# gunesevitan/otto-multi-objective-recommender-system

Measured on AMD Instinct MI355X. Metric: aid-pairs/sec covisitation build, higher is better.
Workload: dtype u64

## Files before the change

otto-multi-objective-recommender-system_amd/csrc/otto_covis.hip:

```cpp
#include "common.h"
#include "topk.h"
#include "scan.h"
#include "../../include/otto_covis.h"

#include <stdarg.h>
#include <string.h>
#include <type_traits>
#include <vector>

namespace otto {

static thread_local std::string g_err;
void set_error(const char* fmt, ...) {
    char buf[1024];
    va_list ap;
    va_start(ap, fmt);
    vsnprintf(buf, sizeof buf, fmt, ap);
    va_end(ap);
    g_err = buf;
}

struct WinPairs {
    const int64_t* off;
    int W;
// ... 1473 lines not shown
__global__ __launch_bounds__(ORD_BLOCK) void k_ord_scatter(const uint64_t* keys, const uint64_t* chunks, uint32_t n, OrdBin dg,
                                                           uint32_t n_blocks, const uint64_t* cell_start, uint64_t* out) {
    __shared__ uint32_t s_bin[ORD_BLOCK];
    const uint32_t i = blockIdx.x * ORD_BLOCK + threadIdx.x;
    const uint32_t bin = i < n ? dg(keys[i]) : 0xffffffffu;
    s_bin[threadIdx.x] = bin;
    __syncthreads();
    if (i >= n) return;
    uint32_t rank = 0;
    for (uint32_t j = 0; j < threadIdx.x; ++j) rank += s_bin[j] == bin ? 1u : 0u;
    const uint64_t pos = cell_start[(size_t)bin * n_blocks + blockIdx.x] + rank;
    if (pos < n) out[pos] = chunks[i];
}

constexpr int N_TOTALS = 18;
constexpr int ITEM_BLOCK_AIDS = 2048;
constexpr int N_ITEM_SCANS = 10;
__global__ __launch_bounds__(256) void k_aid_totals(const uint64_t* cnt64, const uint8_t* boost, const uint32_t* flag, uint32_t n_aids,
                                                    uint32_t l_cap, int allow_packed, unsigned long long* totals,
                                                    unsigned long long* block_part) {
    __shared__ unsigned long long s_t[4][N_TOTALS];
    unsigned long long t[N_TOTALS];
#pragma unroll
    for (int q = 0; q < N_TOTALS; ++q) t[q] = 0;
    const uint32_t x_end = min(n_aids, (blockIdx.x + 1) * (uint32_t)ITEM_BLOCK_AIDS);
    for (uint32_t x = blockIdx.x * ITEM_BLOCK_AIDS + threadIdx.x; x < x_end; x += 256) {
        const uint64_t c64 = cnt64[x], n = c64 & CNT_REC_MASK, r = c64 >> CNT_REC_BITS;
        if (n == 0) continue;
        const int b = n <= (uint64_t)S_CAP ? 0 : (n <= (uint64_t)M_CAP ? 1 : 2);
        t[0] += n; t[1] += r; t[2 + b] += n; t[5 + b] += r;
        ItemCount f{cnt64, boost, flag, b, 0, l_cap, allow_packed, -1};
        const uint64_t items = f((int64_t)x);
        t[8 + b] += items;
        if (b == 2) {
            const int mode = heavy_mode(c64, allow_packed, l_cap);
            t[11 + mode] += items;
            t[14 + mode] += 1;
            ChunkCount cf{cnt64, boost, flag, 0, l_cap, allow_packed};
            t[17] += cf((int64_t)x);
        }
    }
#pragma unroll
    for (int q = 0; q < N_TOTALS; ++q) {
        unsigned long long v = t[q];
        for (int o = 32; o > 0; o >>= 1) v += __shfl_xor(v, o, 64);
        if (lane_id() == 0) s_t[threadIdx.x >> 6][q] = v;
    }
    __syncthreads();
    if (threadIdx.x < N_TOTALS) {
        const unsigned long long v = s_t[0][threadIdx.x] + s_t[1][threadIdx.x] + s_t[2][threadIdx.x] + s_t[3][threadIdx.x];
        if (v) atomicAdd(&totals[threadIdx.x], v);
        if (block_part && threadIdx.x >= N_TOTALS - N_ITEM_SCANS)
            block_part[(size_t)blockIdx.x * N_ITEM_SCANS + threadIdx.x - (N_TOTALS - N_ITEM_SCANS)] = v;
    }
}

struct ItemFillArgs {
    const uint64_t* cnt64;
    const uint8_t* boost;
    uint32_t n_aids;
    uint32_t l_cap;
    int allow_packed;
    const unsigned long long* block_part;
    uint64_t* items[3];
    uint32_t* order[3];
    uint64_t n_pilots[3];
    uint64_t* chunks;
    uint64_t* litem_start;
};
__global__ __launch_bounds__(64 * N_ITEM_SCANS) void k_item_part_scan(unsigned long long* block_part, uint32_t nblk) {
    const int q = threadIdx.x >> 6;
    const unsigned lane = lane_id();
    unsigned long long run = 0;
    for (uint32_t b0 = 0; b0 < nblk; b0 += 64) {
        const uint32_t b = b0 + lane;
        const unsigned long long v = b < nblk ? block_part[(size_t)b * N_ITEM_SCANS + q] : 0ull;
        const unsigned long long inc = wave_incl_scan(v);
        if (b < nblk) block_part[(size_t)b * N_ITEM_SCANS + q] = run + inc - v;
        run += (unsigned long long)__shfl((unsigned long long)inc, 63, 64);
    }
}

__global__ __launch_bounds__(256) void k_items_fill(ItemFillArgs a) {
    __shared__ unsigned long long s_base[N_ITEM_SCANS];
    __shared__ uint64_t s_sc[256 / 64 + 1];
    if (threadIdx.x < N_ITEM_SCANS) s_base[threadIdx.x] = a.block_part[(size_t)blockIdx.x * N_ITEM_SCANS + threadIdx.x];
    __syncthreads();
    uint64_t run[N_ITEM_SCANS];
#pragma unroll
    for (int q = 0; q < N_ITEM_SCANS; ++q) run[q] = s_base[q];
    for (int it = 0; it < ITEM_BLOCK_AIDS / 256; ++it) {
        const uint32_t x = blockIdx.x * ITEM_BLOCK_AIDS + it * 256 + threadIdx.x;
        int b = -1, mode = -1;
        uint64_t items = 0, nch = 0;
        if (x < a.n_aids) {
            const uint64_t c64 = a.cnt64[x], n = c64 & CNT_REC_MASK;
            if (n) {
                b = n <= (uint64_t)S_CAP ? 0 : (n <= (uint64_t)M_CAP ? 1 : 2);
                items = 1;
                if (b == 2) {
                    mode = heavy_mode(c64, a.allow_packed, a.l_cap);
                    const int lg = l_log2r(c64, a.boost[x], a.l_cap, a.allow_packed);
                    items = 1ull << lg;
                    if (lg) nch = ((c64 >> CNT_REC_BITS) + PART_CHUNK_RUNS - 1) / PART_CHUNK_RUNS;
                }
            }
        }
        const uint64_t small = (uint64_t)(b == 0) | (uint64_t)(b == 1) << 12 | (uint64_t)(mode == 0) << 24 | (uint64_t)(mode == 1) << 36 |
                               (uint64_t)(mode == 2) << 48;
        uint64_t tot_small, tot_l, tot_m[3], tot_c;
        const uint64_t ex_small = block_excl_scan<uint64_t, 256>(small, s_sc, &tot_small);
        const uint64_t ex_l = block_excl_scan<uint64_t, 256>(b == 2 ? items : 0ull, s_sc, &tot_l);
        uint64_t ex_m[3];
#pragma unroll
        for (int m = 0; m < 3; ++m) ex_m[m] = block_excl_scan<uint64_t, 256>(mode == m ? items : 0ull, s_sc, &tot_m[m]);
        const uint64_t ex_c = block_excl_scan<uint64_t, 256>(nch, s_sc, &tot_c);
        if (b == 0) a.items[0][run[0] + (ex_small & 0xFFF)] = (uint64_t)x;
        if (b == 1) a.items[1][run[1] + ((ex_small >> 12) & 0xFFF)] = (uint64_t)x;
        const uint64_t s = run[2] + ex_l;
        if (x < a.n_aids) a.litem_start[x] = s;
        if (x == a.n_aids - 1) a.litem_start[a.n_aids] = s + (b == 2 ? items : 0ull);
        if (b == 2) {
            uint64_t lg = 0;
            while ((1ull << lg) < items) ++lg;
            for (uint64_t p = 0; p < items; ++p) a.items[2][s + p] = (uint64_t)x | (p << 26) | (lg << 50);
            const uint64_t r = run[6 + mode] + ((ex_small >> (24 + 12 * mode)) & 0xFFF);
            const uint64_t sm = run[3 + mode] + ex_m[mode];
            uint32_t* ord = a.order[mode];
            ord[r] = (uint32_t)s;
            for (uint64_t p = 1; p < items; ++p) ord[a.n_pilots[mode] + sm + p - r - 1] = (uint32_t)(s + p);
            const uint64_t cs = run[9] + ex_c;
            for (uint64_t q = 0; q < nch; ++q) a.chunks[cs + q] = (uint64_t)x | (q << 26);
        }
        run[0] += tot_small & 0xFFF;
        run[1] += (tot_small >> 12) & 0xFFF;
        run[2] += tot_l;
#pragma unroll
        for (int m = 0; m < 3; ++m) {
            run[6 + m] += (tot_small >> (24 + 12 * m)) & 0xFFF;
            run[3 + m] += tot_m[m];
        }
        run[9] += tot_c;
    }
}

constexpr uint64_t TAB_EMPTY = ~0ull;

struct ItemDesc {
    uint32_t it;
    uint64_t item;
    uint64_t rb, re;
    uint64_t ps, pe;
};

#ifdef OTTO_PHASE_PROF
#define OTTO_PH(i) do { if (threadIdx.x == 0) { const unsigned long long _t = clock64(); ph[i] += _t - ph_t; ph_t = _t; } } while (0)
#else
#define OTTO_PH(i) do {} while (0)
#endif
template <int LOG2T, int THREADS, int GROUP, bool PACKED, int MINW, int GU, int INS_CH, bool DBG>
__global__ __launch_bounds__(THREADS, MINW) void k_reduce(ReduceArgs a) {
    constexpr int T = 1 << LOG2T;
    constexpr int NW = THREADS / 64;
    constexpr bool TP = GROUP == OTTO_COVIS_GROUP_TIME && PACKED;
    using K = typename std::conditional<GROUP == OTTO_COVIS_GROUP_TIME && !PACKED, KeyW, KeyN>::type;
    constexpr bool WIDE = GROUP == OTTO_COVIS_GROUP_TIME && !PACKED;
    auto kw = [](K key) -> uint64_t { if constexpr (TP) return key.c >> REC_AID_BITS; else return kweight(key); };
    constexpr bool DYNAMIC = true;
    constexpr int EXCAP = 64;
    constexpr int PKD = GROUP == OTTO_COVIS_GROUP_TIME ? 1 : PK;
    constexpr bool BOUND = GROUP == OTTO_COVIS_GROUP_TYPE && PKD > 1 && NW == 1;
    constexpr int CCAP = 256;
    constexpr bool HOT = NW > 1 && GROUP == OTTO_COVIS_GROUP_TYPE;
    __shared__ uint64_t s_tab[PACKED ? T : 1];
    __shared__ uint32_t s_key[PACKED ? 1 : T];
    __shared__ uint32_t s_v[3][PACKED ? 1 : T];
    constexpr int OCAP = NW == 1 ? 1 : (LOG2T == 12 ? 1920 : (LOG2T == 14 ? 10240 : (THREADS == 512 ? 4608 : 6144)));
    constexpr int RCAP = OCAP / NW;
    __shared__ uint16_t s_occ[OCAP];
    __shared__ uint32_t s_wcnt[NW];
    __shared__ uint32_t s_hcnt[NW];
    constexpr bool INWAVE = PACKED;
    __shared__ uint16_t s_lbi[(NW > 1 && !INWAVE) ? PKD : 1][(NW > 1 && !INWAVE) ? THREADS : 1];
    __shared__ uint64_t s_exw[(NW > 1 || BOUND) ? PKD : 1][(NW > 1 || BOUND) ? EXCAP : 1];
    __shared__ uint16_t s_cand[BOUND ? CCAP : 1];
    __shared__ uint32_t s_exy[1][(NW > 1 && WIDE) ? EXCAP : 1];
    __shared__ uint64_t s_thrw[PK];
    __shared__ uint32_t s_thry[PK];
    __shared__ uint32_t s_nex[PK];
    __shared__ uint32_t s_more;
    __shared__ uint32_t s_ovf;
    constexpr int LISTCAP = BOUND ? S_CAP : 256;
    __shared__ uint16_t s_list[NW == 1 ? LISTCAP : 1];
    __shared__ uint8_t s_seg[NW * 256 + 32];
    __shared__ ItemDesc s_cur;
    __shared__ ItemDesc s_nxt;

    const int wid = threadIdx.x >> 6;
    const unsigned lane = lane_id();
    constexpr bool HANDOVER = THREADS == M_THREADS;
    const int swid = HANDOVER ? __builtin_amdgcn_readfirstlane(wid) : wid;
    const bool pipe = threadIdx.x == (HANDOVER ? (NW - 1) * 64 : 0);
#ifdef OTTO_PHASE_PROF
    unsigned long long ph[24] = {0, 0, 0, 0, 0, 0, 0, 0, 0, 0, 0, 0, 0, 0, 0, 0, 0, 0, 0, 0, 0, 0, 0, 0}, ph_t = clock64();
#endif

    auto fetch_item = [&](uint32_t idx, ItemDesc& d) {
        d.it = 0xFFFFFFFFu;
        d.item = 0ull;
        if (idx < a.n_work) {
            d.it = a.order ? a.order[idx] : idx;
            d.item = a.items[d.it];
        }
    };
    auto fetch_ranges = [&](ItemDesc& d) {
        d.rb = d.re = d.ps = d.pe = 0;
        if (d.it != 0xFFFFFFFFu) {
            const uint32_t xx = (uint32_t)(d.item & REC_AID_MASK);
            d.rb = a.run_start[xx];
            d.re = a.run_start[xx + 1];
            if ((d.item >> 50) != 0 && a.pstart) {
                d.ps = a.pstart[d.it];
                const uint64_t cap = a.pstart[d.it + 1] - d.ps, got = a.pcursor[d.it];
                d.pe = d.ps + (got < cap ? got : cap);
            }
        }
    };
    ItemDesc cur, nx;
    uint32_t idx_next = 0, idx_far = 0;
    constexpr uint32_t DQ = THREADS == S_THREADS ? 16 : 4;
    uint32_t pool = 0, pool_end = 0, pool_next = 0;
    auto take = [&]() {
        const uint32_t r = pool++;
        if (pool == pool_end) {
            pool = pool_next;
            pool_end = pool + DQ;
            pool_next = atomicAdd(a.work_counter, DQ);
        }
        return r;
    };
    if (DYNAMIC) {
        if (pipe) {
            pool = atomicAdd(a.work_counter, 2 * DQ);
            pool_end = pool + DQ;
            pool_next = pool + DQ;
            const uint32_t i0 = take();
            idx_next = take();
            idx_far = take();
            fetch_item(i0, cur);
            fetch_ranges(cur);
            s_cur = cur;
        }
    } else {
        fetch_item(blockIdx.x, cur);
        fetch_ranges(cur);
    }
    uint32_t sidx = blockIdx.x;
    auto clear_slot = [&](int i) {
        if (PACKED) {
            s_tab[PACKED ? i : 0] = TAB_EMPTY;
        } else {
            s_key[PACKED ? 0 : i] = KEY_EMPTY;
            s_v[0][PACKED ? 0 : i] = 0; s_v[1][PACKED ? 0 : i] = 0; s_v[2][PACKED ? 0 : i] = 0;
        }
    };
    auto clear_table = [&]() {
        for (int i = threadIdx.x; i < T; i += THREADS) clear_slot(i);
    };
    if (NW > 1) {
        clear_table();
        if (threadIdx.x == 0) s_ovf = 0;
    }
    constexpr int BU = GROUP == OTTO_COVIS_GROUP_TIME ? 4 : ((PACKED && THREADS == L_THREADS) ? 12 : 6);
    constexpr bool PREF = THREADS == L_THREADS && GROUP != OTTO_COVIS_GROUP_TIME;
    constexpr bool WARM = (THREADS == L_THREADS || THREADS == 512) && GROUP != OTTO_COVIS_GROUP_TIME;
    uint32_t pre[PREF ? BU : 1];
    bool pre_valid = false;
    auto prefetch_next = [&]() {
        if (!PREF) return;
        const uint64_t nitem = s_nxt.item;
        pre_valid = s_nxt.it != 0xFFFFFFFFu && (nitem >> 50) != 0 && a.pstart != nullptr;
        if (!pre_valid) return;
        const uint64_t ps = s_nxt.ps, pe = s_nxt.pe;
#pragma unroll
        for (int u = 0; u < (PREF ? BU : 1); ++u) {
            const uint64_t i = ps + threadIdx.x + (uint64_t)u * THREADS;
            pre[u] = i < pe ? a.prec[i] : KEY_EMPTY;
        }
    };

    for (;;) {
        if (DYNAMIC) {
            __syncthreads();
            cur = s_cur;
        }
        if (cur.it == 0xFFFFFFFFu) break;
        OTTO_PH(0);
        const uint32_t it = cur.it;
        if (DYNAMIC) {
            if (pipe) fetch_item(idx_next, nx);
#ifdef OTTO_PHASE_PROF
            if (threadIdx.x == 0) { const unsigned long long _t = clock64(); ph[13] += _t - ph_t; }
#endif
        } else {
            fetch_item(sidx + gridDim.x, nx);
        }
        const uint64_t item = cur.item;
        const uint32_t x = (uint32_t)(item & REC_AID_MASK);
        const uint32_t part = (uint32_t)((item >> 26) & 0xFFFFFFu);
        constexpr bool CAN_PART = THREADS != M_THREADS;
        const int lgR = CAN_PART ? (int)(item >> 50) : 0;
        const uint32_t pmask = (1u << lgR) - 1u;
        const int pshift = 32 - LOG2T - lgR;

        K guess[PKD];
        const bool use_guess = NW > 1 && lgR > 0 && a.tau_w != nullptr;
#pragma unroll
        for (int j = 0; j < PKD; ++j) {
            kclear(guess[j]);
            if (use_guess && j < (BOUND ? 1 : a.nk)) {
                const size_t o = (size_t)j * a.n_aids + x;
                kload(guess[j], a.tau_w[o], WIDE ? a.tau_y[o] : 0u);
            }
        }
        if (NW == 1 && !(DBG && (a.debug_skip & 4))) clear_table();
        if (NW == 1) {
            s_ovf = 0;
            wave_lds_sync();
        }
        OTTO_PH(1);

        auto probe_step = [&](uint32_t y) -> uint32_t { return (((y * 0x85EBCA6Bu) ^ (y >> 7)) * 0xC2B2AE35u >> (32 - LOG2T)) | 1u; };
        uint32_t wc = 0;
        auto note_new = [&](uint64_t m, uint32_t slot) {
            if (NW == 1) return;
            if (m == 0) return;
            const uint32_t pos = wc + __builtin_amdgcn_mbcnt_hi((uint32_t)(m >> 32), __builtin_amdgcn_mbcnt_lo((uint32_t)m, 0u));
            if (__builtin_amdgcn_inverse_ballot_w64(m) && pos < (uint32_t)RCAP) s_occ[NW > 1 ? wid * RCAP + pos : 0] = (uint16_t)slot;
            wc += (uint32_t)__popcll(m);
        };
        constexpr int ICMP_EQ = 32, ICMP_NE = 33;
        auto probe_on = [&](uint32_t y, uint32_t slot, unsigned long long add, unsigned long long fresh) -> uint32_t {
            const uint32_t step = probe_step(y);
            for (int probe = 1; probe < T; ++probe) {
                slot = (slot + step) & (T - 1);
                const unsigned long long old = atomicCAS((unsigned long long*)&s_tab[PACKED ? slot : 0], (unsigned long long)TAB_EMPTY, fresh | add);
                if (old == TAB_EMPTY) return slot;
                if ((uint32_t)(old >> 36) == y) {
                    atomicAdd((unsigned long long*)&s_tab[PACKED ? slot : 0], add);
                    return 0xFFFFFFFFu;
                }
            }
            s_ovf = 1;
            return 0xFFFFFFFFu;
        };
        auto wide_add = [&](uint32_t rc, uint32_t found, uint32_t e) {
            if (GROUP == OTTO_COVIS_GROUP_TIME) {
                atomicAdd(&s_v[0][PACKED ? 0 : found], 1u);
                const uint32_t old = atomicAdd(&s_v[1][PACKED ? 0 : found], e);
                if (old + e < old) atomicAdd(&s_v[2][PACKED ? 0 : found], 1u);
            } else if (GROUP == OTTO_COVIS_GROUP_TYPE) {
                const uint32_t tyj = (rc >> REC_AID_BITS) & 3u;
                if (tyj < 3u) atomicAdd(&s_v[tyj][PACKED ? 0 : found], 1u);
            } else {
                const uint32_t fb = (rc >> 28) >> a.chan_shift;
                if (fb & 1u) atomicAdd(&s_v[0][PACKED ? 0 : found], 1u);
                if (fb & 2u) atomicAdd(&s_v[1][PACKED ? 0 : found], 1u);
                if (fb & 4u) atomicAdd(&s_v[2][PACKED ? 0 : found], 1u);
            }
        };
        auto packed_add = [&](uint32_t rc, uint32_t e) -> unsigned long long {
            uint32_t add0, add1, add2;
            if (GROUP == OTTO_COVIS_GROUP_TIME) {
                return 65536ull + (unsigned long long)e;
            } else if (GROUP == OTTO_COVIS_GROUP_TYPE) {
                const uint32_t tyj = (rc >> REC_AID_BITS) & 3u;
                return (unsigned long long)((1u << ((tyj * 12u) & 31u)) & 0x01001001u);
            } else {
                const uint32_t fb = (rc >> 28) >> a.chan_shift;
                add0 = fb & 1u; add1 = (fb >> 1) & 1u; add2 = (fb >> 2) & 1u;
            }
            return (unsigned long long)add0 | ((unsigned long long)add1 << 12) | ((unsigned long long)add2 << 24);
        };
        auto insert_batch = [&](auto ntag, const uint32_t* rc, const uint64_t* okin, const uint32_t* e) {
            constexpr int N = decltype(ntag)::value;
            constexpr int CH = INS_CH;
            if (DBG && (a.debug_skip & 8)) {
#pragma unroll
                for (int u = 0; u < N; ++u)
                    if (__builtin_amdgcn_inverse_ballot_w64(okin[u]) && rc[u] == 0xDEADBEEFu) s_ovf = 1;
                return;
            }
#pragma unroll
            for (int c0 = 0; c0 < N; c0 += CH) {
                bool ok[CH];
                uint64_t okm[CH];
                uint64_t any = 0;
#pragma unroll
                for (int q = 0; q < CH; ++q) {
                    const int u = c0 + q;
                    uint64_t m = u < N ? okin[u < N ? u : 0] : 0ull;
                    if (GROUP == OTTO_COVIS_GROUP_FILTER) m &= __builtin_amdgcn_uicmp(((rc[u < N ? u : 0] >> 28) >> a.chan_shift) & 7u, 0u, ICMP_NE);
                    okm[q] = m;
                    ok[q] = __builtin_amdgcn_inverse_ballot_w64(m);
                    any |= m;
                }
                if (any == 0) continue;
                if (PACKED) {
                    uint32_t oldhi[CH];
                    unsigned long long addq[CH];
#pragma unroll
                    for (int q = 0; q < CH; ++q) {
                        const uint32_t r = rc[c0 + q < N ? c0 + q : 0];
                        const uint32_t slot = rec_hash(r) >> (32 - LOG2T);
                        oldhi[q] = 0xFFFFFFFFu;
                        addq[q] = packed_add(r, e[c0 + q < N ? c0 + q : 0]);
                        if (ok[q]) {
                            const unsigned long long o = atomicCAS((unsigned long long*)&s_tab[PACKED ? slot : 0], (unsigned long long)TAB_EMPTY,
                                                                   ((unsigned long long)(r & REC_AID_MASK) << 36) | addq[q]);
                            oldhi[q] = (uint32_t)(o >> 32);
                        }
                        note_new(okm[q] & __builtin_amdgcn_uicmp(oldhi[q], 0xFFFFFFFFu, ICMP_EQ), slot);
                    }
#pragma unroll
                    for (int q = 0; q < CH; ++q) {
                        const uint32_t r = rc[c0 + q < N ? c0 + q : 0];
                        const uint32_t y = r & REC_AID_MASK, slot = rec_hash(r) >> (32 - LOG2T);
                        uint32_t late = 0xFFFFFFFFu;
                        if (oldhi[q] != 0xFFFFFFFFu) {
                            if ((oldhi[q] >> 4) == y) atomicAdd((unsigned long long*)&s_tab[PACKED ? slot : 0], addq[q]);
                            else late = probe_on(y, slot, addq[q], (unsigned long long)y << 36);
                        }
                        note_new(__builtin_amdgcn_uicmp(late, 0xFFFFFFFFu, ICMP_NE), late);
                    }
                    continue;
                }
                uint32_t old[CH];
#pragma unroll
                for (int q = 0; q < CH; ++q) {
                    const uint32_t r = rc[c0 + q < N ? c0 + q : 0];
                    old[q] = KEY_EMPTY;
                    if (ok[q]) old[q] = atomicCAS(&s_key[PACKED ? 0 : rec_hash(r) >> (32 - LOG2T)], KEY_EMPTY, r & REC_AID_MASK);
                    note_new(okm[q] & __builtin_amdgcn_uicmp(old[q], KEY_EMPTY, ICMP_EQ), rec_hash(r) >> (32 - LOG2T));
                }
#pragma unroll
                for (int q = 0; q < CH; ++q) {
                    const uint32_t r = rc[c0 + q < N ? c0 + q : 0];
                    const uint32_t y = r & REC_AID_MASK;
                    uint32_t sl = rec_hash(r) >> (32 - LOG2T);
                    uint32_t late = 0xFFFFFFFFu;
                    if (ok[q]) {
                        bool found = old[q] == KEY_EMPTY || old[q] == y;
                        const uint32_t step = probe_step(y);
                        for (int probe = 1; !found && probe < T; ++probe) {
                            sl = (sl + step) & (T - 1);
                            const uint32_t o2 = atomicCAS(&s_key[PACKED ? 0 : sl], KEY_EMPTY, y);
                            if (o2 == KEY_EMPTY) late = sl;
                            found = o2 == KEY_EMPTY || o2 == y;
                        }
                        if (!found) s_ovf = 1;
                        else wide_add(r, sl, e[c0 + q < N ? c0 + q : 0]);
                    }
                    note_new(__builtin_amdgcn_uicmp(late, 0xFFFFFFFFu, ICMP_NE), late);
                }
            }
        };

        auto slot_keys = [&](int i, K (&out)[PKD]) {
            uint32_t y, v0, v1, v2;
            if (PACKED) {
                const uint64_t v = s_tab[i];
                y = v == TAB_EMPTY ? KEY_EMPTY : (uint32_t)(v >> 36);
                v0 = (uint32_t)v & 0xFFFu; v1 = (uint32_t)(v >> 12) & 0xFFFu; v2 = (uint32_t)(v >> 24) & 0xFFFu;
            } else {
                y = s_key[i];
                v0 = s_v[0][i]; v1 = s_v[1][i]; v2 = s_v[2][i];
// ... 239 lines not shown
                        uint16_t sl = 0;
                        if (li < nvalid) {
                            K kl, kh;
                            sl = s_list[NW == 1 ? li : 0];
                            slot_lohi((int)sl, kl, kh);
                            c = !kbetter(thr, kh);
                        }
                        const uint64_t m = __ballot(c);
                        const uint32_t pos = ncand + __builtin_amdgcn_mbcnt_hi((uint32_t)(m >> 32), __builtin_amdgcn_mbcnt_lo((uint32_t)m, 0u));
                        if (c && pos < (uint32_t)CCAP) s_cand[pos] = sl;
                        ncand += (uint32_t)__popcll(m);
                    }
                    overflow = ncand > (uint32_t)CCAP;
                }
                wave_lds_sync();
                for (int j = 0; j < a.nk; ++j) {
                    if (overflow) wave_exact_topk(j);
                    else finish_kind(j, ncand);
                }
                wave_lds_sync();
            }
        }
        OTTO_PH(4);
        } else if constexpr (NW == 1) {
        bool fast_done = false;
        OTTO_PH(7);
        if (fast_done || (DBG && (a.debug_skip & 2))) {
        } else if (ovf) {
            if (threadIdx.x == 0) {
                a.flag[x] = 1;
                a.boost[x] = (uint8_t)(lgR - l_log2r(a.cnt64[x], 0, a.l_cap, a.allow_packed) + 1);
                atomicAdd(a.ovf_count, 1u);
            }
        } else {
            constexpr int MPL = T / THREADS;
            static_assert(MPL <= 32, "consumed-slot bitmask is 32 bits");
            bool compact_done = false;
            if (NW == 1) {
                uint32_t nvalid = 0;
#pragma unroll
                for (int q = 0; q < MPL; ++q) {
                    const int i = q * THREADS + threadIdx.x;
                    const bool v = PACKED ? (s_tab[PACKED ? i : 0] != TAB_EMPTY) : (s_key[PACKED ? 0 : i] != KEY_EMPTY);
                    const uint64_t m = __ballot(v);
                    const uint32_t pos = nvalid + __builtin_amdgcn_mbcnt_hi((uint32_t)(m >> 32), __builtin_amdgcn_mbcnt_lo((uint32_t)m, 0u));
                    if (v && pos < (uint32_t)LISTCAP) s_list[pos] = (uint16_t)i;
                    nvalid += (uint32_t)__popcll(m);
                }
                auto select_from_registers = [&](auto mtag) {
                    constexpr int MC = decltype(mtag)::value;
                    __syncthreads();
                    K c[PKD][MC];
#pragma unroll
                    for (int q = 0; q < MC; ++q) {
                        K kk[PKD];
#pragma unroll
                        for (int j = 0; j < PKD; ++j) kclear(kk[j]);
                        const uint32_t li = (uint32_t)q * 64u + lane;
                        if (li < nvalid) slot_keys((int)s_list[li], kk);
#pragma unroll
                        for (int j = 0; j < PKD; ++j) c[j][q] = kk[j];
                    }
                    K bests[PKD];
                    wave_topk_select_multi<MC, PKD, K>(c, a.nk, a.k, bests);
#pragma unroll
                    for (int j = 0; j < PKD; ++j)
                        if (j < a.nk) emit(j, bests[j]);
                    compact_done = true;
                    __syncthreads();
                };
                if (nvalid > 64u && nvalid <= 128u) select_from_registers(std::integral_constant<int, 2>{});
                else if (nvalid > 128u && nvalid <= 256u) select_from_registers(std::integral_constant<int, 4>{});
                if (nvalid <= 64u) {
                    __syncthreads();
                    K bests[PKD];
#pragma unroll
                    for (int j = 0; j < PKD; ++j) kclear(bests[j]);
                    if (lane < nvalid) slot_keys((int)s_list[lane], bests);
                    wave_bitonic_sort_multi<PKD, K>(bests);
#pragma unroll
                    for (int j = 0; j < PKD; ++j)
                        if (j < a.nk) emit(j, bests[j]);
                    compact_done = true;
                    __syncthreads();
                }
            }
            if (!compact_done) {
            K lb[PKD];
            uint32_t done[PKD];
            uint32_t nonempty = 0;
            {
                int bi[PKD];
#pragma unroll
                for (int j = 0; j < PKD; ++j) { kclear(lb[j]); bi[j] = 0; }
#pragma unroll 2
                for (int q = 0; q < MPL; ++q) {
                    K kk[PKD];
                    slot_keys(q * THREADS + threadIdx.x, kk);
                    bool any = false;
#pragma unroll
                    for (int j = 0; j < PKD; ++j) {
                        any = any || kvalid(kk[j]);
                        if (kbetter(kk[j], lb[j])) { lb[j] = kk[j]; bi[j] = q; }
                    }
                    if (any) nonempty |= 1u << q;
                }
#pragma unroll
                for (int j = 0; j < PKD; ++j) done[j] = 1u << bi[j];
            }
            if (NW == 1) {
                K bests[PKD];
#pragma unroll
                for (int j = 0; j < PKD; ++j) bests[j] = lb[j];
                wave_bitonic_sort_multi<PKD, K>(bests);
                for (;;) {
                    K thr[PKD], cb[PKD];
                    int ci[PKD];
#pragma unroll
                    for (int j = 0; j < PKD; ++j) {
                        thr[j] = kshfl(bests[j], a.k - 1);
                        kclear(cb[j]);
                        ci[j] = -1;
                    }
#pragma unroll 1
                    for (int q = 0; q < MPL; ++q) {
                        K kk[PKD];
                        slot_keys(q * THREADS + threadIdx.x, kk);
#pragma unroll
                        for (int j = 0; j < PKD; ++j)
                            if (!((done[j] >> q) & 1u) && kvalid(kk[j]) && kbetter(kk[j], thr[j]) &&
                                (ci[j] < 0 || kbetter(kk[j], cb[j]))) { cb[j] = kk[j]; ci[j] = q; }
                    }
                    bool any = false;
#pragma unroll
                    for (int j = 0; j < PKD; ++j) {
                        if (j >= a.nk) continue;
                        const bool qual = ci[j] >= 0;
                        if (__ballot(qual) == 0) continue;
                        any = true;
                        if (qual) done[j] |= 1u << ci[j];
                        wave_topk_push(bests[j], cb[j], a.k);
                    }
                    if (!any) break;
                }
#pragma unroll
                for (int j = 0; j < PKD; ++j)
                    if (j < a.nk) emit(j, bests[j]);
            }
            }
        }
        } else {
        const uint32_t nocc = s_wcnt[NW > 1 ? wid : 0];
        bool dense = true;
#pragma unroll
        for (int w = 0; w < NW; ++w) dense = dense && s_wcnt[NW > 1 ? w : 0] <= (uint32_t)RCAP;
        uint32_t nwalk = nocc;
        bool hot = false;
        if (HOT && dense && a.hot_ok) {
            constexpr int NITMAX = (RCAP + 63) / 64;
            uint32_t ent[NITMAX];
            uint32_t hv = 0, vv = 0;
            const int nq = (int)((nocc + 63u) / 64u);
#pragma unroll
            for (int q = 0; q < NITMAX; ++q) {
                const uint32_t idx = (uint32_t)q * 64u + lane;
                ent[q] = 0;
                if (q < nq && idx < nocc) {
                    const uint32_t sl = s_occ[NW > 1 ? wid * RCAP + idx : 0];
                    ent[q] = sl;
                    vv |= 1u << q;
                    bool light;
                    if (PACKED) light = (s_tab[PACKED ? sl : 0] & 0xFFFFFFFFFull) == 1ull;
                    else light = s_v[0][PACKED ? 0 : sl] == 1u && (s_v[1][PACKED ? 0 : sl] | s_v[2][PACKED ? 0 : sl]) == 0u;
                    if (!light) hv |= 1u << q;
                }
            }
            uint32_t H = 0;
#pragma unroll
            for (int q = 0; q < NITMAX; ++q)
                if (q < nq) H += (uint32_t)__popcll(__ballot((hv >> q) & 1u));
            uint32_t hpos = 0, lpos = H;
#pragma unroll
            for (int q = 0; q < NITMAX; ++q) {
                if (q < nq) {
                    const bool v = (vv >> q) & 1u, h = (hv >> q) & 1u;
                    const uint64_t mh = __ballot(h), ml = __ballot(v && !h);
                    if (v) {
                        const uint64_t m = h ? mh : ml;
                        const uint32_t pos = (h ? hpos : lpos) + __builtin_amdgcn_mbcnt_hi((uint32_t)(m >> 32), __builtin_amdgcn_mbcnt_lo((uint32_t)m, 0u));
                        s_occ[NW > 1 ? wid * RCAP + pos : 0] = (uint16_t)ent[q];
                    }
                    hpos += (uint32_t)__popcll(mh);
                    lpos += (uint32_t)__popcll(ml);
                }
            }
            if (lane == 0) s_hcnt[NW > 1 ? wid : 0] = H;
            wave_lds_sync();
            nwalk = H;
            hot = true;
        }
        if (ovf) {
            if (threadIdx.x == 0) {
                a.flag[x] = 1;
                a.boost[x] = (uint8_t)(lgR - l_log2r(a.cnt64[x], 0, a.l_cap, a.allow_packed) + 1);
                atomicAdd(a.ovf_count, 1u);
            }
        } else if (!(DBG && (a.debug_skip & 2))) {
            constexpr int MPL = T / THREADS;
            int nit = dense ? (int)((nwalk + 63u) / 64u) : MPL;
            auto slot_at = [&](int q) -> int {
                if (!dense) return q * THREADS + (int)threadIdx.x;
                const uint32_t idx = (uint32_t)q * 64u + lane;
                return idx < nwalk ? (int)s_occ[NW > 1 ? wid * RCAP + idx : 0] : -1;
            };
            auto slot_key1 = [&](int i, uint32_t c0, uint32_t c1, uint32_t c2) {
                uint32_t y, v0, v1, v2;
                if (PACKED) {
                    const uint64_t v = s_tab[PACKED ? i : 0];
                    y = v == TAB_EMPTY ? KEY_EMPTY : (uint32_t)(v >> 36);
                    v0 = (uint32_t)v & 0xFFFu; v1 = (uint32_t)(v >> 12) & 0xFFFu; v2 = (uint32_t)(v >> 24) & 0xFFFu;
                } else {
                    y = s_key[PACKED ? 0 : i];
                    v0 = s_v[0][PACKED ? 0 : i]; v1 = s_v[1][PACKED ? 0 : i]; v2 = s_v[2][PACKED ? 0 : i];
                }
                uint64_t uw = 0, qw = 0;
                if (y != KEY_EMPTY) {
                    if (TP) uw = (uint64_t)v0 | ((uint64_t)v1 << 12) | ((uint64_t)v2 << 24);
                    else if (GROUP == OTTO_COVIS_GROUP_TIME) qw = 65536ull * v0 + (((uint64_t)v2 << 32) | v1);
                    else if (PACKED) uw = __umul24(v0, c0) + __umul24(v1, c1) + __umul24(v2, c2);
                    else uw = (uint64_t)v0 * c0 + (uint64_t)v1 * c1 + (uint64_t)v2 * c2;
                }
                K r;
                kmake(r, uw, qw, y);
                return r;
            };
            auto emit_ranked = [&](int j, K key, uint32_t rank, int nv) {
                const bool put = kvalid(key) && rank < (uint32_t)a.k;
                if (lgR == 0) {
                    const size_t o = ((size_t)(a.kind_base + j) * a.n_aids + x) * (size_t)a.k + rank;
                    if (put) { a.out_y[o] = kaid(key); a.out_w[o] = kw(key); }
                    if (lane == 0) a.out_n[(size_t)(a.kind_base + j) * a.n_aids + x] = nv < a.k ? nv : a.k;
                } else {
                    const size_t base = ((size_t)it * a.nk + j) * (size_t)a.k;
                    if (put) kstore(key, &a.part_w[base + rank], &a.part_y[base + rank]);
                    if ((int)lane < a.k && (int)lane >= nv) { K z; kclear(z); kstore(z, &a.part_w[base + lane], &a.part_y[base + lane]); }
                }
            };
            auto finish_list = [&](int j, uint32_t n, bool store_tau) {
                K key;
                kclear(key);
                if (lane < n) kload(key, s_exw[j][lane], s_exy[0][WIDE ? lane : 0]);
                uint32_t rank = 0;
#pragma unroll 4
                for (uint32_t i = 0; i < n; ++i) {
                    K o;
                    kload(o, s_exw[j][i], s_exy[0][WIDE ? i : 0]);
                    kcount_better(rank, o, key);
                }
                emit_ranked(j, key, rank, (int)n);
                if (store_tau && n >= 32u && kvalid(key) && rank == 31u) ktau_store(key, a.tau_w, a.tau_y, (size_t)j * a.n_aids + x);
            };
            auto wave_exact_topk = [&](int j) {
                const uint32_t c0 = a.coef[j][0], c1 = a.coef[j][1], c2 = a.coef[j][2];
                const int nreg = dense ? NW : 1;
                K lb;
                kclear(lb);
                int bi = -1;
                for (int w = 0; w < nreg; ++w) {
                    const int total = dense ? (int)(hot ? s_hcnt[NW > 1 ? w : 0] : s_wcnt[NW > 1 ? w : 0]) : T;
                    for (int i = (int)lane; i < total; i += 64) {
                        const int sl = dense ? (int)s_occ[NW > 1 ? w * RCAP + i : 0] : i;
                        const K key = slot_key1(sl, c0, c1, c2);
                        if (kbetter(key, lb)) { lb = key; bi = sl; }
                    }
                }
                K best = lb;
                wave_bitonic_sort_desc(best);
                for (int w = 0; w < nreg; ++w) {
                    const int total = dense ? (int)(hot ? s_hcnt[NW > 1 ? w : 0] : s_wcnt[NW > 1 ? w : 0]) : T;
                    for (int i0 = 0; i0 < total; i0 += 64) {
                        const int i = i0 + (int)lane;
                        K key;
                        kclear(key);
                        if (i < total) {
                            const int sl = dense ? (int)s_occ[NW > 1 ? w * RCAP + i : 0] : i;
                            if (sl != bi) key = slot_key1(sl, c0, c1, c2);
                        }
                        wave_topk_push(best, key, a.k);
                    }
                }
                emit(j, best);
            };
            auto append = [&](int j, K key) {
                const uint32_t pos = atomicAdd(&s_nex[j], 1u);
                if (pos < (uint32_t)EXCAP) kstore(key, &s_exw[j][pos], &s_exy[0][WIDE ? pos : 0]);
                else s_more = 1;
            };

            bool fast_done = false;
            bool pre_issued = false;
            constexpr bool SH = HOT && NW <= 4;
            constexpr int SHR = 4;
            if (SH && hot && a.hot_ok >= 2) {
                __syncthreads();
                uint32_t pre[NW + 1];
                pre[0] = 0;
#pragma unroll
                for (int w = 0; w < NW; ++w) pre[w + 1] = pre[w] + s_hcnt[NW > 1 ? w : 0];
                const uint32_t th = pre[NW];
                if (th < (uint32_t)a.k) {
                    hot = false;
                    nwalk = nocc;
                    nit = (int)((nwalk + 63u) / 64u);
                } else if (th <= 64u * SHR) {
#ifdef OTTO_PHASE_PROF
                    if (threadIdx.x == 0) ph[14]++;
#endif
#ifdef OTTO_PHASE_PROF
                    const unsigned long long sel_t = clock64();
#endif
                    if (swid < nsel) {
                        const int j = swid;
                        const uint32_t c0 = a.coef[j][0], c1 = a.coef[j][1], c2 = a.coef[j][2];
                        K keys[SHR], lbk;
                        kclear(lbk);
#pragma unroll
                        for (int q = 0; q < SHR; ++q) {
                            const uint32_t e = (uint32_t)q * 64u + lane;
                            kclear(keys[q]);
                            if (e < th) {
                                int w = 0;
#pragma unroll
                                for (int ww = 1; ww < NW; ++ww)
                                    if (e >= pre[ww]) w = ww;
                                const uint32_t sl = s_occ[NW > 1 ? w * RCAP + (int)(e - pre[w]) : 0];
                                keys[q] = slot_key1((int)sl, c0, c1, c2);
                                if (kbetter(keys[q], lbk)) lbk = keys[q];
                            }
                        }
                        kstore(lbk, &s_exw[j][lane], &s_exy[0][WIDE ? lane : 0]);
                        wave_lds_sync();
                        uint32_t rank = 0;
#pragma unroll 8
                        for (int i = 0; i < 64; ++i) {
                            K o;
                            kload(o, s_exw[j][i], s_exy[0][WIDE ? i : 0]);
                            kcount_better(rank, o, lbk);
                        }
                        const uint64_t mk = __ballot(kvalid(lbk) && rank == (uint32_t)(a.k - 1));
                        K thr;
                        kclear(thr);
                        if (mk) thr = kshfl(lbk, __ffsll((unsigned long long)mk) - 1);
                        wave_lds_sync();
                        uint32_t n = 0;
#pragma unroll
                        for (int q = 0; q < SHR; ++q) {
                            const bool c = kvalid(keys[q]) && !kbetter(thr, keys[q]);
                            const uint64_t m = __ballot(c);
                            const uint32_t pos = n + __builtin_amdgcn_mbcnt_hi((uint32_t)(m >> 32), __builtin_amdgcn_mbcnt_lo((uint32_t)m, 0u));
                            if (c && pos < (uint32_t)EXCAP) kstore(keys[q], &s_exw[j][pos], &s_exy[0][WIDE ? pos : 0]);
                            n += (uint32_t)__popcll(m);
                        }
                        wave_lds_sync();
                        if (n > (uint32_t)EXCAP) wave_exact_topk(j);
                        else finish_list(j, n, false);
                    } else if (swid == NW - 1) {
                        warm_next();
                    }
#ifdef OTTO_PHASE_PROF
                    if (threadIdx.x == 0) ph[18] += clock64() - sel_t;
#endif
                    fast_done = true;
                }
            }
            bool gv = use_guess && !fast_done;
#pragma unroll
            for (int j = 0; j < PKD; ++j)
                if (j < a.nk && !kvalid(guess[j])) gv = false;
            if (gv) {
                if (threadIdx.x < PK) s_nex[threadIdx.x] = 0;
                if (threadIdx.x == 0) s_more = 0;
                if (WARM && pipe) s_nxt = nx;
                __syncthreads();
                uint32_t warm = 0;
                if (WARM && s_nxt.it != 0xFFFFFFFFu && (s_nxt.item >> 50) != 0 && a.pstart != nullptr) {
                    const uint64_t wi = s_nxt.ps + (uint64_t)threadIdx.x * 16u;
                    if (wi < s_nxt.pe) warm = a.prec[wi];
                }
                for (int q = 0; q < nit; ++q) {
                    const int sl = slot_at(q);
                    if (sl < 0) continue;
                    K kk[PKD];
                    slot_keys(sl, kk);
#pragma unroll
                    for (int j = 0; j < PKD; ++j)
                        if (j < a.nk && kvalid(kk[j]) && kbetter(kk[j], guess[j])) append(j, kk[j]);
                }
                asm volatile("" :: "v"(warm));
                __syncthreads();
                prefetch_next();
                pre_issued = true;
                bool ok = s_more == 0;
#pragma unroll
                for (int j = 0; j < PKD; ++j)
                    if (j < a.nk && s_nex[j] < (uint32_t)a.k) ok = false;
#ifdef OTTO_PHASE_PROF
                if (threadIdx.x == 0) { ph[8]++; if (ok) ph[9]++; else if (s_more) ph[11]++; else ph[10]++; }
#endif
                if (ok) {
#ifdef OTTO_PHASE_PROF
                    const unsigned long long sel_t = clock64();
#endif
                    if (wid < a.nk && wid < PKD) finish_list(wid, s_nex[wid], true);
#ifdef OTTO_PHASE_PROF
                    if (threadIdx.x == 0) ph[18] += clock64() - sel_t;
#endif
                    fast_done = true;
                }
                __syncthreads();
            }
            OTTO_PH(7);
            if (!fast_done) {
                K lb[PKD];
                int bi[PKD];
                constexpr int NCK = (PACKED && THREADS <= 512) ? 3 : 0;
                K ck[NCK > 0 ? NCK : 1][PKD];
                for (;;) {
#pragma unroll
                for (int j = 0; j < PKD; ++j) { kclear(lb[j]); bi[j] = 0xFFFF; }
#pragma unroll
                for (int q = 0; q < NCK; ++q) {
                    const int sl = q < nit ? slot_at(q) : -1;
#pragma unroll
                    for (int j = 0; j < PKD; ++j) kclear(ck[q][j]);
                    if (sl >= 0) {
                        slot_keys(sl, ck[q]);
#pragma unroll
                        for (int j = 0; j < PKD; ++j)
                            if (kbetter(ck[q][j], lb[j])) { lb[j] = ck[q][j]; bi[j] = sl; }
                    }
                }
                for (int q = NCK; q < nit; ++q) {
                    const int sl = slot_at(q);
                    if (sl < 0) continue;
                    K kk[PKD];
                    slot_keys(sl, kk);
#pragma unroll
                    for (int j = 0; j < PKD; ++j)
                        if (kbetter(kk[j], lb[j])) { lb[j] = kk[j]; bi[j] = sl; }
                }
#pragma unroll
                for (int j = 0; j < PKD; ++j) {
                    if (!INWAVE) {
                        if (j < a.nk) s_lbi[!INWAVE ? j : 0][(NW > 1 && !INWAVE) ? threadIdx.x : 0] = (uint16_t)bi[j];
                        continue;
                    }
                    K g = lb[j];
#pragma unroll
                    for (int m = 1; m < NW; m <<= 1) {
                        const K o = kshfl_xor(g, m);
                        if (kbetter(o, g)) g = o;
                    }
                    if (j < a.nk && (lane & (NW - 1)) == 0) {
                        const int gi = wid * (64 / NW) + (int)(lane / NW);
                        kstore(g, &s_exw[j][gi], &s_exy[0][WIDE ? gi : 0]);
                    }
                }
                if (threadIdx.x < PK) s_nex[threadIdx.x] = 0;
                if (threadIdx.x == 0) s_more = 0;
                __syncthreads();
                if (hot) {
                    uint32_t th = 0;
#pragma unroll
                    for (int w = 0; w < NW; ++w) th += s_hcnt[NW > 1 ? w : 0];
                    if (th < (uint32_t)a.k) {
                        hot = false;
                        nwalk = nocc;
                        nit = (int)((nwalk + 63u) / 64u);
                        continue;
                    }
                }
                break;
                }
                OTTO_PH(4);
                if (swid >= nsel) {
                    if (swid == NW - 1) warm_next();
                } else {
                    const int j = swid;
                    K gb;
                    if (INWAVE) {
                        kload(gb, s_exw[j][lane], s_exy[0][WIDE ? lane : 0]);
                    } else {
                        kclear(gb);
                        const uint32_t c0 = a.coef[j][0], c1 = a.coef[j][1], c2 = a.coef[j][2];
#pragma unroll
                        for (int q = 0; q < NW; ++q) {
                            const uint32_t sl = s_lbi[!INWAVE ? j : 0][(NW > 1 && !INWAVE) ? q * 64 + lane : 0];
                            if (sl != 0xFFFFu) {
                                const K o = slot_key1((int)sl, c0, c1, c2);
                                if (kbetter(o, gb)) gb = o;
                            }
                        }
                        kstore(gb, &s_exw[j][lane], &s_exy[0][WIDE ? lane : 0]);
                        wave_lds_sync();
                    }
                    uint32_t rank = 0;
#pragma unroll 8
                    for (int i = 0; i < 64; ++i) {
                        K o;
                        kload(o, s_exw[j][i], s_exy[0][WIDE ? i : 0]);
                        kcount_better(rank, o, gb);
                    }
                    const uint64_t mk = __ballot(kvalid(gb) && rank == (uint32_t)(a.k - 1));
                    K thr;
                    kclear(thr);
                    if (mk) thr = kshfl(gb, __ffsll((unsigned long long)mk) - 1);
                    if (lane == 0) kstore(thr, &s_thrw[j], &s_thry[j]);
                    if (use_guess && kvalid(gb) && rank == 31u) ktau_store(gb, a.tau_w, a.tau_y, (size_t)j * a.n_aids + x);
                    wave_lds_sync();
                }
                OTTO_PH(5);
                __syncthreads();
                K thr[PKD];
#pragma unroll
                for (int j = 0; j < PKD; ++j) kload(thr[j], s_thrw[j], s_thry[j]);
#pragma unroll
                for (int q = 0; q < NCK; ++q) {
#pragma unroll
                    for (int j = 0; j < PKD; ++j)
                        if (j < a.nk && kvalid(ck[q][j]) && !kbetter(thr[j], ck[q][j])) append(j, ck[q][j]);
                }
                for (int q = NCK; q < nit; ++q) {
                    const int sl = slot_at(q);
                    if (sl < 0) continue;
                    K kk[PKD];
                    slot_keys(sl, kk);
#pragma unroll
                    for (int j = 0; j < PKD; ++j)
                        if (j < a.nk && kvalid(kk[j]) && !kbetter(thr[j], kk[j])) append(j, kk[j]);
                }
                if (PREF && !pre_issued && pipe) s_nxt = nx;
                __syncthreads();
                if (!pre_issued) prefetch_next();
                OTTO_PH(6);
                if (wid < a.nk && wid < PKD) {
                    if (s_more) wave_exact_topk(wid);
                    else finish_list(wid, s_nex[wid] < (uint32_t)EXCAP ? s_nex[wid] : (uint32_t)EXCAP, false);
                }
                OTTO_PH(7);
            }
        }
        __syncthreads();
#ifdef OTTO_PHASE_PROF
        const unsigned long long clr_t = clock64();
#endif
        if (!(DBG && (a.debug_skip & 4))) {
            if (dense) {
                for (uint32_t idx = lane; idx < nocc; idx += 64u) clear_slot((int)s_occ[NW > 1 ? wid * RCAP + idx : 0]);
            } else {
                clear_table();
            }
        }
        if (threadIdx.x == 0) s_ovf = 0;
#ifdef OTTO_PHASE_PROF
        if (threadIdx.x == 0) ph[17] += clock64() - clr_t;
#endif
        }

        if (DYNAMIC) {
            __syncthreads();
            if (pipe) {
                s_cur = nx;
                idx_next = idx_far;
                idx_far = take();
            }
        } else {
            cur = nx;
            sidx += gridDim.x;
        }
    }
#ifdef OTTO_PHASE_PROF
    if (threadIdx.x == 0 && a.prof)
        for (int i = 0; i < 24; ++i) atomicAdd(&a.prof[i], ph[i]);
#endif
}

template <typename K, bool RAW>
__device__ __forceinline__ void merge_lists(const ReduceArgs& a, uint32_t it, uint32_t x, int lgR, int j, unsigned lane) {
    const uint64_t ncand = (uint64_t)a.k << lgR;
    auto fetch = [&](uint64_t c0) {
        const uint64_t c = c0 + lane;
        K cand;
        kclear(cand);
        if (c < ncand) {
            const size_t o = ((size_t)(it + c / a.k) * a.nk + j) * (size_t)a.k + (c % a.k);
            kload(cand, a.part_w[o], a.part_y[o]);
        }
        return cand;
    };
    K best;
    kclear(best);
    K cand = fetch(0);
    for (uint64_t c0 = 0; c0 < ncand; c0 += 64) {
        const K nxt = c0 + 64 < ncand ? fetch(c0 + 64) : cand;
        if (c0 == 0) { best = cand; wave_bitonic_sort_desc(best); }
        else wave_topk_push(best, cand, a.k);
        cand = nxt;
    }
    const bool valid = (int)lane < a.k && kvalid(best);
    const size_t o = ((size_t)(a.kind_base + j) * a.n_aids + x) * (size_t)a.k + lane;
    if (valid) {
        a.out_y[o] = kaid(best);
        if constexpr (RAW) a.out_w[o] = best.c >> REC_AID_BITS;
        else a.out_w[o] = kweight(best);
    }
    const int nvalid = __popcll(__ballot(valid));
    if (lane == 0) a.out_n[(size_t)(a.kind_base + j) * a.n_aids + x] = nvalid;
}

template <int GROUP>
__global__ __launch_bounds__(64 * PK) void k_merge(ReduceArgs a) {
    const uint32_t it = blockIdx.x;
    if (it >= a.n_items) return;
    const uint64_t item = a.items[it];
    const uint32_t part = (uint32_t)((item >> 26) & 0xFFFFFFu);
    const int lgR = (int)(item >> 50);
    if (part != 0 || lgR == 0) return;
    const uint32_t x = (uint32_t)(item & REC_AID_MASK);
    if (a.flag[x]) return;
    const unsigned lane = lane_id();
    const int j = (int)(threadIdx.x >> 6);
    if (j >= a.nk) return;
    if constexpr (GROUP == OTTO_COVIS_GROUP_TIME) {
        if (heavy_mode(a.cnt64[x], a.allow_packed, a.l_cap) != 0) merge_lists<KeyN, true>(a, it, x, lgR, j, lane);
        else merge_lists<KeyW, false>(a, it, x, lgR, j, lane);
    } else {
        merge_lists<KeyN, false>(a, it, x, lgR, j, lane);
    }
}

struct ExportRuns {
    const uint32_t* run_x;
    const uint64_t* run_desc;
    uint32_t lo, hi;
    __device__ uint64_t operator()(int64_t i) const {
        const uint32_t x = run_x[i];
        return (desc_len(run_desc[i]) && x >= lo && x < hi) ? 1ull : 0ull;
    }
};
struct ExportRecs {
    const uint32_t* run_x;
    const uint64_t* run_desc;
    uint32_t lo, hi;
    __device__ uint64_t operator()(int64_t i) const {
        const uint32_t x = run_x[i];
        const uint64_t len = desc_pairs(run_desc[i]);
        return (len && x >= lo && x < hi) ? len : 0ull;
    }
};

__global__ void k_export(const uint32_t* run_x, const uint64_t* run_desc, int64_t n_slots, uint32_t lo, uint32_t hi,
                         const uint64_t* run_pos, const uint64_t* rec_pos, const uint32_t* rec, const uint32_t* tw,
                         uint32_t* o_hdr, uint32_t* o_rec, uint32_t* o_tw) {
    for (int64_t i = (int64_t)blockIdx.x * blockDim.x + threadIdx.x; i < n_slots; i += (int64_t)gridDim.x * blockDim.x) {
        const uint64_t d = run_desc[i];
        const uint32_t len = desc_pairs(d), sp = desc_sp(d);
        const uint32_t x = run_x[i];
        if (len && x >= lo && x < hi) {
            const uint64_t rp = run_pos[i], cp = rec_pos[i], off = desc_slot(d);
            o_hdr[2 * rp] = x;
            o_hdr[2 * rp + 1] = len;
            for (uint32_t t = 0; t < len; ++t) {
                const uint32_t pos = t >= sp ? t + 1 : t;
                o_rec[cp + t] = rec[off + pos];
                if (o_tw) o_tw[cp + t] = tw[off + (sp != DESC_SP_NONE ? sp : pos)];
            }
        }
    }
}

constexpr int MAX_OWNERS = 64;
struct OwnerArgs {
    const uint32_t* run_x;
    const uint64_t* run_desc;
    int64_t slot0;
    int64_t n_slots;
    int n_owners;
    uint32_t bounds[MAX_OWNERS + 1];
    uint64_t run_base[MAX_OWNERS];
    uint64_t rec_base[MAX_OWNERS];
    unsigned long long* totals;
    const uint32_t* rec;
    const uint32_t* tw;
    uint32_t* o_hdr;
    uint32_t* o_rec;
    uint32_t* o_tw;
};

__device__ __forceinline__ int owner_of(const OwnerArgs& a, uint32_t x) {
    int o = 0;
    while (o + 1 < a.n_owners && x >= a.bounds[o + 1]) ++o;
    return o;
}

constexpr int EXP_REC_BITS = 34;

__global__ __launch_bounds__(256) void k_export_plan(OwnerArgs a) {
    __shared__ unsigned long long s_tot[MAX_OWNERS];
    if (threadIdx.x < MAX_OWNERS) s_tot[threadIdx.x] = 0;
    __syncthreads();
    for (int64_t i = (int64_t)blockIdx.x * 256 + threadIdx.x; i < a.n_slots; i += (int64_t)gridDim.x * 256) {
        const uint64_t d = a.run_desc[a.slot0 + i];
        const uint32_t len = desc_pairs(d);
        if (len) atomicAdd(&s_tot[owner_of(a, a.run_x[a.slot0 + i])], (1ull << EXP_REC_BITS) | len);
    }
    __syncthreads();
    if ((int)threadIdx.x < a.n_owners && s_tot[threadIdx.x]) atomicAdd(&a.totals[threadIdx.x], s_tot[threadIdx.x]);
}

constexpr int EXP_CHUNK = 512;
__global__ __launch_bounds__(256) void k_export_fill(OwnerArgs a) {
    constexpr int PER = EXP_CHUNK / 256;
    __shared__ unsigned long long s_rr[MAX_OWNERS];
    __shared__ unsigned long long s_rbase[MAX_OWNERS], s_cbase[MAX_OWNERS];
    __shared__ uint64_t s_src[EXP_CHUNK], s_dst[EXP_CHUNK];
// ... 1121 lines not shown
```

Baseline: 61.29 billion.

## Double-buffer item descriptors, taper work chunks, and clear table early in idle waves

Replaces the single shared current/next item descriptors with a parity-indexed double buffer so multi-wave blocks drop a barrier per item. The slot is also shrunk when partitions are unused. Work-queue chunk size now tapers as remaining work drops, to reduce tail imbalance. Guess thresholds are loaded once by a few threads into shared memory and broadcast via readfirstlane. Waves that are not selecting top-k clear the hash table early, overlapping the clear with selection and skipping a barrier. This adds more complex synchronization, and a missed publish or clear path could corrupt results.

```diff
diff --git a/otto-multi-objective-recommender-system_amd/csrc/otto_covis.hip b/otto-multi-objective-recommender-system_amd/csrc/otto_covis.hip
--- a/otto-multi-objective-recommender-system_amd/csrc/otto_covis.hip
+++ b/otto-multi-objective-recommender-system_amd/csrc/otto_covis.hip
@@ -1649,6 +1649,21 @@
     uint64_t rb, re;
     uint64_t ps, pe;
 };
+template <bool PARTS> struct ItemSlot {
+    ItemDesc d;
+    __device__ __forceinline__ void put(const ItemDesc& s) { d = s; }
+    __device__ __forceinline__ ItemDesc get() const { return d; }
+};
+template <> struct ItemSlot<false> {
+    uint64_t item, rb, re;
+    __device__ __forceinline__ void put(const ItemDesc& s) { item = s.it == 0xFFFFFFFFu ? ~0ull : s.item; rb = s.rb; re = s.re; }
+    __device__ __forceinline__ ItemDesc get() const {
+        ItemDesc s;
+        s.it = item == ~0ull ? 0xFFFFFFFFu : 0u;
+        s.item = item; s.rb = rb; s.re = re; s.ps = s.pe = 0;
+        return s;
+    }
+};
 
 #ifdef OTTO_PHASE_PROF
 #define OTTO_PH(i) do { if (threadIdx.x == 0) { const unsigned long long _t = clock64(); ph[i] += _t - ph_t; ph_t = _t; } } while (0)
@@ -1690,14 +1705,14 @@
     constexpr int LISTCAP = BOUND ? S_CAP : 256;
     __shared__ uint16_t s_list[NW == 1 ? LISTCAP : 1];
     __shared__ uint8_t s_seg[NW * 256 + 32];
-    __shared__ ItemDesc s_cur;
-    __shared__ ItemDesc s_nxt;
+    __shared__ ItemSlot<THREADS != M_THREADS> s_desc[NW > 1 ? 2 : 1];
+    uint32_t par = 0;
 
     const int wid = threadIdx.x >> 6;
     const unsigned lane = lane_id();
     constexpr bool HANDOVER = THREADS == M_THREADS;
     const int swid = HANDOVER ? __builtin_amdgcn_readfirstlane(wid) : wid;
-    const bool pipe = threadIdx.x == (HANDOVER ? (NW - 1) * 64 : 0);
+    const bool pipe = threadIdx.x == (NW > 1 ? (NW - 1) * 64 : 0);
 #ifdef OTTO_PHASE_PROF
     unsigned long long ph[24] = {0, 0, 0, 0, 0, 0, 0, 0, 0, 0, 0, 0, 0, 0, 0, 0, 0, 0, 0, 0, 0, 0, 0, 0}, ph_t = clock64();
 #endif
@@ -1726,27 +1741,32 @@
     ItemDesc cur, nx;
     uint32_t idx_next = 0, idx_far = 0;
     constexpr uint32_t DQ = THREADS == S_THREADS ? 16 : 4;
-    uint32_t pool = 0, pool_end = 0, pool_next = 0;
+    constexpr uint32_t DQ_MIN = THREADS == S_THREADS ? 8 : 1;
+    const uint32_t taper_shift = 32u - (uint32_t)__builtin_clz(2u * gridDim.x - 1u);
+    uint32_t pool = 0, pool_next = 0, pool_cn = DQ | DQ << 16;
     auto take = [&]() {
         const uint32_t r = pool++;
-        if (pool == pool_end) {
+        --pool_cn;
+        if ((pool_cn & 0xFFFFu) == 0) {
             pool = pool_next;
-            pool_end = pool + DQ;
-            pool_next = atomicAdd(a.work_counter, DQ);
+            const uint32_t left = a.n_work > pool ? a.n_work - pool : 0u;
+            uint32_t n = left >> taper_shift;
+            n = n < DQ_MIN ? DQ_MIN : (n > DQ ? DQ : n);
+            pool_cn = pool_cn >> 16 | n << 16;
+            pool_next = atomicAdd(a.work_counter, n);
         }
         return r;
     };
     if (DYNAMIC) {
         if (pipe) {
             pool = atomicAdd(a.work_counter, 2 * DQ);
-            pool_end = pool + DQ;
             pool_next = pool + DQ;
             const uint32_t i0 = take();
             idx_next = take();
             idx_far = take();
             fetch_item(i0, cur);
             fetch_ranges(cur);
-            s_cur = cur;
+            s_desc[0].put(cur);
         }
     } else {
         fetch_item(blockIdx.x, cur);
@@ -1775,10 +1795,11 @@
     bool pre_valid = false;
     auto prefetch_next = [&]() {
         if (!PREF) return;
-        const uint64_t nitem = s_nxt.item;
-        pre_valid = s_nxt.it != 0xFFFFFFFFu && (nitem >> 50) != 0 && a.pstart != nullptr;
+        const ItemDesc nxt = s_desc[NW > 1 ? par ^ 1 : 0].get();
+        const uint64_t nitem = nxt.item;
+        pre_valid = nxt.it != 0xFFFFFFFFu && (nitem >> 50) != 0 && a.pstart != nullptr;
         if (!pre_valid) return;
-        const uint64_t ps = s_nxt.ps, pe = s_nxt.pe;
+        const uint64_t ps = nxt.ps, pe = nxt.pe;
 #pragma unroll
         for (int u = 0; u < (PREF ? BU : 1); ++u) {
             const uint64_t i = ps + threadIdx.x + (uint64_t)u * THREADS;
@@ -1786,10 +1807,15 @@
         }
     };
 
+    if (DYNAMIC && NW > 1) {
+        __syncthreads();
+        cur = s_desc[0].get();
+    }
+    bool published = false;
     for (;;) {
-        if (DYNAMIC) {
+        if (DYNAMIC && NW == 1) {
             __syncthreads();
-            cur = s_cur;
+            cur = s_desc[0].get();
         }
         if (cur.it == 0xFFFFFFFFu) break;
         OTTO_PH(0);
@@ -1813,12 +1839,12 @@
         K guess[PKD];
         const bool use_guess = NW > 1 && lgR > 0 && a.tau_w != nullptr;
 #pragma unroll
-        for (int j = 0; j < PKD; ++j) {
-            kclear(guess[j]);
-            if (use_guess && j < (BOUND ? 1 : a.nk)) {
-                const size_t o = (size_t)j * a.n_aids + x;
-                kload(guess[j], a.tau_w[o], WIDE ? a.tau_y[o] : 0u);
-            }
+        for (int j = 0; j < PKD; ++j) kclear(guess[j]);
+        if (use_guess && (int)threadIdx.x < a.nk && (int)threadIdx.x < PKD) {
+            const size_t o = (size_t)threadIdx.x * a.n_aids + x;
+            K g;
+            kload(g, a.tau_w[o], WIDE ? a.tau_y[o] : 0u);
+            kstore(g, &s_thrw[threadIdx.x], &s_thry[threadIdx.x]);
         }
         if (NW == 1 && !(DBG && (a.debug_skip & 4))) clear_table();
         if (NW == 1) {
@@ -2364,6 +2390,7 @@
         } else {
         const uint32_t nocc = s_wcnt[NW > 1 ? wid : 0];
         bool dense = true;
+        bool cleared = false;
 #pragma unroll
         for (int w = 0; w < NW; ++w) dense = dense && s_wcnt[NW > 1 ? w : 0] <= (uint32_t)RCAP;
         uint32_t nwalk = nocc;
@@ -2509,6 +2536,15 @@
                 else s_more = 1;
             };
 
+            constexpr bool EARLY = PACKED && THREADS == L_THREADS;
+            auto clear_early = [&]() {
+                for (int w = wid - nsel; w < NW; w += NW - nsel) {
+                    const uint32_t cnt = s_wcnt[NW > 1 ? w : 0];
+                    for (uint32_t idx = lane; idx < cnt; idx += 64u) clear_slot((int)s_occ[NW > 1 ? w * RCAP + idx : 0]);
+                }
+                if (threadIdx.x == (NW - 1) * 64) s_ovf = 0;
+            };
+            const bool can_early = EARLY && dense && !(DBG && (a.debug_skip & 4));
             bool fast_done = false;
             bool pre_issued = false;
             constexpr bool SH = HOT && NW <= 4;
@@ -2585,6 +2621,16 @@
                     fast_done = true;
                 }
             }
+            if (use_guess) {
+#pragma unroll
+                for (int j = 0; j < PKD; ++j) {
+                    if (j >= a.nk) continue;
+                    const uint64_t w = s_thrw[j];
+                    const uint32_t y = s_thry[j];
+                    kload(guess[j], ((uint64_t)(uint32_t)__builtin_amdgcn_readfirstlane((int)(uint32_t)(w >> 32)) << 32) |
+                                    (uint32_t)__builtin_amdgcn_readfirstlane((int)(uint32_t)w), (uint32_t)__builtin_amdgcn_readfirstlane((int)y));
+                }
+            }
             bool gv = use_guess && !fast_done;
 #pragma unroll
             for (int j = 0; j < PKD; ++j)
@@ -2592,12 +2638,15 @@
             if (gv) {
                 if (threadIdx.x < PK) s_nex[threadIdx.x] = 0;
                 if (threadIdx.x == 0) s_more = 0;
-                if (WARM && pipe) s_nxt = nx;
+                if (WARM && pipe) { s_desc[NW > 1 ? par ^ 1 : 0].put(nx); published = true; }
                 __syncthreads();
                 uint32_t warm = 0;
-                if (WARM && s_nxt.it != 0xFFFFFFFFu && (s_nxt.item >> 50) != 0 && a.pstart != nullptr) {
-                    const uint64_t wi = s_nxt.ps + (uint64_t)threadIdx.x * 16u;
-                    if (wi < s_nxt.pe) warm = a.prec[wi];
+                if (WARM) {
+                    const ItemDesc nxt = s_desc[NW > 1 ? par ^ 1 : 0].get();
+                    if (nxt.it != 0xFFFFFFFFu && (nxt.item >> 50) != 0 && a.pstart != nullptr) {
+                        const uint64_t wi = nxt.ps + (uint64_t)threadIdx.x * 16u;
+                        if (wi < nxt.pe) warm = a.prec[wi];
+                    }
                 }
                 for (int q = 0; q < nit; ++q) {
                     const int sl = slot_at(q);
@@ -2623,13 +2672,16 @@
 #ifdef OTTO_PHASE_PROF
                     const unsigned long long sel_t = clock64();
 #endif
-                    if (wid < a.nk && wid < PKD) finish_list(wid, s_nex[wid], true);
+                    if (wid < nsel) finish_list(wid, s_nex[wid], true);
+                    else if (can_early) clear_early();
 #ifdef OTTO_PHASE_PROF
                     if (threadIdx.x == 0) ph[18] += clock64() - sel_t;
 #endif
                     fast_done = true;
-                }
-                __syncthreads();
+                    cleared = can_early;
+                } else {
+                    __syncthreads();
+                }
             }
             OTTO_PH(7);
             if (!fast_done) {
@@ -2751,17 +2803,23 @@
                     for (int j = 0; j < PKD; ++j)
                         if (j < a.nk && kvalid(kk[j]) && !kbetter(thr[j], kk[j])) append(j, kk[j]);
                 }
-                if (PREF && !pre_issued && pipe) s_nxt = nx;
+                if (PREF && !pre_issued && pipe) { s_desc[NW > 1 ? par ^ 1 : 0].put(nx); published = true; }
                 __syncthreads();
                 if (!pre_issued) prefetch_next();
                 OTTO_PH(6);
-                if (wid < a.nk && wid < PKD) {
-                    if (s_more) wave_exact_topk(wid);
+                const bool more = s_more != 0;
+                if (wid < nsel) {
+                    if (more) wave_exact_topk(wid);
                     else finish_list(wid, s_nex[wid] < (uint32_t)EXCAP ? s_nex[wid] : (uint32_t)EXCAP, false);
-                }
+                } else if (!more && can_early) {
+                    clear_early();
+                }
+                cleared = !more && can_early;
                 OTTO_PH(7);
             }
         }
+        if (pipe && !published) s_desc[NW > 1 ? par ^ 1 : 0].put(nx);
+        if (!cleared) {
         __syncthreads();
 #ifdef OTTO_PHASE_PROF
         const unsigned long long clr_t = clock64();
@@ -2778,11 +2836,17 @@
         if (threadIdx.x == 0) ph[17] += clock64() - clr_t;
 #endif
         }
+        }
 
         if (DYNAMIC) {
             __syncthreads();
+            if (NW > 1) {
+                par ^= 1;
+                cur = s_desc[NW > 1 ? par : 0].get();
+                published = false;
+            }
             if (pipe) {
-                s_cur = nx;
+                if (NW == 1) s_desc[0].put(nx);
                 idx_next = idx_far;
                 idx_far = take();
             }
```

Result: no change. 61.67 billion (median of 6 runs) (+0.6%).
